# ltinphan/convex-mpc-unitree-go2

Measured on AMD Instinct MI355X. Metric: batched QP solves/sec (N=16, 4-leg friction cone) at 1/2/4/8 MI355X, higher is better.
Workload: dtype f32

## Files before the change

### convex-mpc-unitree-go2_amd/csrc/cmpc_condense.h

```cpp
#pragma once
#include "cmpc_instance.h"

namespace cmpc {

template <int NC>
__device__ __forceinline__ void condense_finish(Smem<NC>& s, f4 (&M)[Cfg<NC>::NTL], int n,
                                                float shift) {
  using C = Cfg<NC>;
  const int lane = opaque_lane();
  const int g = lane >> 4, c = lane & 15;
#pragma unroll
  for (int I = 0; I < C::TT; ++I) {
#pragma unroll
    for (int J = 0; J <= I; ++J) {
      if (J != I && 16 * I + 16 <= n) continue;
      f4 v = M[tile_index(I, J)];
      const int col = 16 * J + c;
#pragma unroll
      for (int q = 0; q < 4; ++q) {
        const int row = 16 * I + 4 * g + q;
        if (row >= n || col >= n) v[q] = (row == col) ? 1.f : 0.f;
        else if (row == col) v[q] += s.Rt[row] + shift;
      }
      M[tile_index(I, J)] = v;
    }
  }
  WSYNC();
}

__device__ __forceinline__ int lane_state(int c) {
  return ((c & 3) < 3) ? 3 * (c >> 2) + (c & 3) : -1;
}
template <class SM>
__device__ __forceinline__ void state_operands(SM& s, int g, int c, float (&aA)[3],
                                               float (&aT)[3], f4& q2) {
  const int sc = lane_state(c);
  q2 = f4{0.f, 0.f, 0.f, 0.f};
#pragma unroll
  for (int q = 0; q < 3; ++q) {
    const int r = 3 * g + q;
    aA[q] = (sc >= 0) ? s.A[sc * 12 + r] : 0.f;
    aT[q] = (sc >= 0) ? s.A[r * 12 + sc] : 0.f;
    q2[q] = (r == sc) ? s.Q2[r] : 0.f;
  }
}

template <class SM>
__device__ __forceinline__ void blockrow_C_chunk(SM& s, float* Cs, const f4& Pt, int J, int p0,
                                                 int p1, int n, int g, int c) {
  const int p = 16 * J + c;
  float bt[3];
#pragma unroll
  for (int q = 0; q < 3; ++q) bt[q] = s.Bt[p * kBS + 3 * g + q];
  f4 d = {0.f, 0.f, 0.f, 0.f};
#pragma unroll
  for (int q = 0; q < 3; ++q) d = mfma4(Pt[q], (p < n) ? bt[q] : 0.f, d);
  if (p >= p0 && p < p1) {
#pragma unroll
    for (int q = 0; q < 3; ++q) Cs[p * 12 + 3 * g + q] = d[q];
  }
}
__device__ __forceinline__ void blockrow_P_step(f4& Pt, const float (&aT)[3], const f4& q2) {
  f4 y = {0.f, 0.f, 0.f, 0.f}, z = {0.f, 0.f, 0.f, 0.f};
#pragma unroll
  for (int q = 0; q < 3; ++q) y = mfma4(Pt[q], aT[q], y);
#pragma unroll
  for (int q = 0; q < 3; ++q) z = mfma4(aT[q], y[q], z);
#pragma unroll
  for (int q = 0; q < 4; ++q) Pt[q] = z[q] + q2[q];
}

template <int NC>
__device__ __forceinline__ void condense_tiles_fwd(Smem<NC>& s, const KParams& P,
                                                   f4 (&M)[Cfg<NC>::NTL], int n, float shift) {
  using C = Cfg<NC>;
  const int lane = opaque_lane();
  const int g = lane >> 4, c = lane & 15;
  const int N = P.N;
  n = uniform(n);
#pragma unroll
  for (int t = 0; t < C::NTL; ++t) M[t] = f4{0.f, 0.f, 0.f, 0.f};
  float aA[3], q2[3];
  const int sc = lane_state(c);
#pragma unroll
  for (int q = 0; q < 3; ++q) {
    const int r = 3 * g + q;
    aA[q] = (sc >= 0) ? s.A[sc * 12 + r] : 0.f;
    q2[q] = s.Q2[r];
  }
  int kI[C::TT];
#pragma unroll
  for (int I = 0; I < C::TT; ++I) kI[I] = (16 * I < n) ? s.par[16 * I] : N;
  f4 Gd[C::TT];
#pragma unroll
  for (int J = 0; J < C::TT; ++J) Gd[J] = f4{0.f, 0.f, 0.f, 0.f};
  for (int t = 0; t < N; ++t) {
    if (t > 0) {
#pragma unroll
      for (int J = 0; J < C::TT; ++J) {
        if (kI[J] >= t) continue;
        f4 d = {0.f, 0.f, 0.f, 0.f};
#pragma unroll
        for (int q = 0; q < 3; ++q) d = mfma4(aA[q], Gd[J][q], d);
        Gd[J] = d;
      }
    }
    const int p0 = s.off[t], p1 = s.off[t + 1];
#pragma unroll
    for (int J = 0; J < C::TT; ++J) {
      if (16 * J + 15 < p0 || 16 * J >= p1) continue;
      const int p = 16 * J + c;
      if (p >= p0 && p < p1) {
        const float* bp = &s.Bt[p * kBS + 3 * g];
        Gd[J] = f4{bp[0], bp[1], bp[2], 0.f};
      }
    }
#pragma unroll
    for (int I = 0; I < C::TT; ++I) {
      if (kI[I] > t) continue;
      float a[3];
#pragma unroll
      for (int q = 0; q < 3; ++q) a[q] = q2[q] * Gd[I][q];
#pragma unroll
      for (int J = 0; J <= I; ++J) {
        f4 acc = M[tile_index(I, J)];
#pragma unroll
        for (int q = 0; q < 3; ++q) acc = mfma4(a[q], Gd[J][q], acc);
        M[tile_index(I, J)] = acc;
      }
    }
  }
  condense_finish<NC>(s, M, n, shift);
}

template <int NC>
__device__ __forceinline__ void mirror_diagonals(Smem<NC>& s, f4 (&M)[Cfg<NC>::NTL], int n, int N) {
  using C = Cfg<NC>;
  const int lane = opaque_lane();
  const int g = lane >> 4, c = lane & 15;
  WSYNC();
  float* T = s.G;
#pragma unroll
  for (int I = 0; I < C::TT; ++I) {
    if (16 * I >= n) continue;
    f4 v = M[tile_index(I, I)];
#pragma unroll
    for (int q = 0; q < 4; ++q) T[(4 * g + q) * 16 + c] = v[q];
    WSYNC();
    const int pc = 16 * I + c;
    const int kc = (pc < n) ? s.par[pc] : N;
#pragma unroll
    for (int q = 0; q < 4; ++q) {
      const int pr = 16 * I + 4 * g + q;
      const int kr = (pr < n) ? s.par[pr] : N;
      if (kc > kr) v[q] = T[c * 16 + 4 * g + q];
    }
    M[tile_index(I, I)] = v;
    WSYNC();
  }
}

template <int NC>
__device__ __forceinline__ void condense_tiles_bc(Smem<NC>& s, const KParams& P,
                                                  f4 (&M)[Cfg<NC>::NTL], int n, float shift) {
  using C = Cfg<NC>;
  const int lane = opaque_lane();
  const int g = lane >> 4, c = lane & 15;
  const int N = P.N;
  n = uniform(n);
#pragma unroll
  for (int t = 0; t < C::NTL; ++t) M[t] = f4{0.f, 0.f, 0.f, 0.f};
  float aA[3], aT[3];
  f4 q2;
  state_operands(s, g, c, aA, aT, q2);
  float* Cs = s.G;
  f4 Pt = q2;
  WSYNC();
  for (int i = N - 1; i >= 0; --i) {
    const int p0 = s.off[i], p1 = s.off[i + 1];
#pragma unroll
    for (int J = 0; J < C::TT; ++J) {
      if (16 * J + 15 < p0 || 16 * J >= p1) continue;
      blockrow_C_chunk(s, Cs, Pt, J, p0, p1, n, g, c);
    }
    if (i > 0) blockrow_P_step(Pt, aT, q2);
  }
  WSYNC();
  int kI[C::TT];
#pragma unroll
  for (int I = 0; I < C::TT; ++I) kI[I] = (16 * I < n) ? s.par[16 * I] : N;
  f4 Gd[C::TT];
#pragma unroll
  for (int J = 0; J < C::TT; ++J) Gd[J] = f4{0.f, 0.f, 0.f, 0.f};
  for (int t = 0; t < N; ++t) {
    if (t > 0) {
#pragma unroll
      for (int J = 0; J < C::TT; ++J) {
        if (kI[J] >= t) continue;
        f4 d = {0.f, 0.f, 0.f, 0.f};
#pragma unroll
        for (int q = 0; q < 3; ++q) d = mfma4(aA[q], Gd[J][q], d);
        Gd[J] = d;
      }
    }
    const int p0 = s.off[t], p1 = s.off[t + 1];
#pragma unroll
    for (int J = 0; J < C::TT; ++J) {
      if (16 * J + 15 < p0 || 16 * J >= p1) continue;
      const int p = 16 * J + c;
      if (p >= p0 && p < p1) {
        const float* bp = &s.Bt[p * kBS + 3 * g];
        Gd[J] = f4{bp[0], bp[1], bp[2], 0.f};
      }
    }
#pragma unroll
    for (int I = 0; I < C::TT; ++I) {
      if (16 * I + 15 < p0 || 16 * I >= p1) continue;
      const int p = 16 * I + c;
      float a[3] = {0.f, 0.f, 0.f};
      if (p >= p0 && p < p1) {
#pragma unroll
        for (int q = 0; q < 3; ++q) a[q] = Cs[p * 12 + 3 * g + q];
      }
#pragma unroll
      for (int J = 0; J <= I; ++J) {
        f4 acc = M[tile_index(I, J)];
#pragma unroll
        for (int q = 0; q < 3; ++q) acc = mfma4(a[q], Gd[J][q], acc);
        M[tile_index(I, J)] = acc;
      }
    }
  }
  mirror_diagonals<NC>(s, M, n, N);
  condense_finish<NC>(s, M, n, shift);
}

__device__ __forceinline__ void step_sums(int k, int N, float& S0, float& S1, float& S2) {
  S0 = (float)(N - k);
  S1 = (float)((N * (N - 1) - k * (k - 1)) >> 1);
  S2 = (float)(((N - 1) * N * (2 * N - 1) - (k - 1) * k * (2 * k - 1)) / 6);
}

template <int NC>
__device__ __forceinline__ void condense_tiles_nil(Smem<NC>& s, const KParams& P,
                                                   f4 (&M)[Cfg<NC>::NTL], int n, float shift) {
  using C = Cfg<NC>;
  const int lane = opaque_lane();
  const int g = lane >> 4, c = lane & 15;
  const int N = P.N;
  n = uniform(n);
  const int TA = (n + 15) >> 4;
#pragma unroll
  for (int t = 0; t < C::NTL; ++t) M[t] = f4{0.f, 0.f, 0.f, 0.f};
  float* Vs = s.G;
  {
    const int sc = lane_state(c);
    float aN[3];
#pragma unroll
    for (int q = 0; q < 3; ++q) {
      const int r = 3 * g + q;
      aN[q] = (sc >= 0) ? s.A[sc * 12 + r] - ((sc == r) ? 1.f : 0.f) : 0.f;
    }
    WSYNC();
#pragma unroll
    for (int J = 0; J < C::TT; ++J) {
      if (J >= TA) continue;
      const int p = 16 * J + c;
      float bt[3];
#pragma unroll
      for (int q = 0; q < 3; ++q) bt[q] = (p < n) ? s.Bt[p * kBS + 3 * g + q] : 0.f;
      f4 d = {0.f, 0.f, 0.f, 0.f};
#pragma unroll
      for (int q = 0; q < 3; ++q) d = mfma4(aN[q], bt[q], d);
#pragma unroll
      for (int q = 0; q < 3; ++q) Vs[p * 12 + 3 * g + q] = d[q];
    }
  }
  WSYNC();
  float q2[3];
#pragma unroll
  for (int q = 0; q < 3; ++q) q2[q] = s.Q2[3 * g + q];
  float uc[C::TT][3], vc[C::TT][3];
#pragma unroll
  for (int J = 0; J < C::TT; ++J) {
    const int p = 16 * J + c;
    const bool ok = J < TA && p < n;
    const float kf = ok ? (float)s.par[p] : 0.f;
#pragma unroll
    for (int q = 0; q < 3; ++q) {
      vc[J][q] = ok ? Vs[p * 12 + 3 * g + q] : 0.f;
      uc[J][q] = ok ? fmaf(-kf, vc[J][q], s.Bt[p * kBS + 3 * g + q]) : 0.f;
    }
  }
#pragma unroll
  for (int I = 0; I < C::TT; ++I) {
    if (I >= TA) continue;
    float x[3], y[3];
    {
      const int p = 16 * I + c;
      const bool ok = p < n;
      const int k = ok ? s.par[p] : 0;
      const float kf = (float)k;
      float S0, S1, S2;
      step_sums(k, N, S0, S1, S2);
#pragma unroll
      for (int q = 0; q < 3; ++q) {
        const float v = ok ? Vs[p * 12 + 3 * g + q] : 0.f;
        const float u = ok ? fmaf(-kf, v, s.Bt[p * kBS + 3 * g + q]) : 0.f;
        x[q] = q2[q] * fmaf(S0, u, S1 * v);
        y[q] = q2[q] * fmaf(S1, u, S2 * v);
      }
    }
#pragma unroll
    for (int J = 0; J <= I; ++J) {
      float u[3], v[3];
#pragma unroll
      for (int q = 0; q < 3; ++q) {
        u[q] = uc[J][q];
        v[q] = vc[J][q];
      }
      f4 acc = M[tile_index(I, J)];
#pragma unroll
      for (int q = 0; q < 3; ++q) acc = mfma4(x[q], u[q], acc);
#pragma unroll
      for (int q = 0; q < 3; ++q) acc = mfma4(y[q], v[q], acc);
      M[tile_index(I, J)] = acc;
    }
  }
  mirror_diagonals<NC>(s, M, n, N);
  condense_finish<NC>(s, M, n, shift);
}

template <class SM>
__device__ __forceinline__ bool nilpotent_step(SM& s) {
  const int lane = opaque_lane();
  WSYNC();
  bool nz = false;
#pragma unroll
  for (int e0 = 0; e0 < 144; e0 += 64) {
    const int e = e0 + lane;
    if (e < 144) {
      const int i = e / 12, j = e % 12;
      float acc = 0.f;
#pragma unroll
      for (int k = 0; k < 12; ++k) {
        const float nik = s.A[i * 12 + k] - ((i == k) ? 1.f : 0.f);
        const float nkj = s.A[k * 12 + j] - ((k == j) ? 1.f : 0.f);
        acc = fmaf(nik, nkj, acc);
      }
      nz |= acc != 0.f;
    }
  }
  return __any(nz) == 0;
}

template <int NC>
__device__ __forceinline__ void condense_tiles(Smem<NC>& s, const KParams& P,
                                               f4 (&M)[Cfg<NC>::NTL], int n, float shift,
                                               bool nil = false) {
  if (nil) {
    condense_tiles_nil<NC>(s, P, M, n, shift);
    return;
  }
  if constexpr (NC <= 128) {
    if (P.latency_mode) {
      condense_tiles_bc<NC>(s, P, M, n, shift);
      return;
    }
  }
  condense_tiles_fwd<NC>(s, P, M, n, shift);
}

}
```

### convex-mpc-unitree-go2_amd/csrc/cmpc_factor.h

```cpp
#pragma once
#include "cmpc_instance.h"

namespace cmpc {

constexpr int kSweepPipeMaxNC = 128;
template <int NC, int K, class SM>
__device__ __forceinline__ void sweep_publish(SM& s, const f4 (&M)[Cfg<NC>::NTL], int sub,
                                              int g, int c) {
  using C = Cfg<NC>;
  const int c0 = 4 * sub;
  const int pc = c - c0;
  const bool colw = pc >= 0 && pc < 4;
  if (colw) {
#pragma unroll
    for (int I = K; I < C::TT; ++I) {
      f4 m = M[tile_index(I, K)];
      if (I == K) {
#pragma unroll
        for (int q = 0; q < 4; ++q) m[q] -= (4 * g + q == c) ? 1.f : 0.f;
      }
#pragma unroll
      for (int q = 0; q < 4; ++q) s.pan[(16 * I + 4 * g + q) * 4 + pc] = m[q];
    }
  }
  WSYNC();
}

__device__ __forceinline__ void pivot_block(const float (&Dm)[16], int g, float& w0, float& w1,
                                            float& w2, float& w3, float& ig) {
  const bool g1 = g == 1, g2 = g == 2, g3 = g == 3;
  const float i0 = __builtin_amdgcn_rcpf(Dm[0]);
  const float l10 = Dm[4] * i0, l20 = Dm[8] * i0, l30 = Dm[12] * i0;
  const float i1 = __builtin_amdgcn_rcpf(Dm[5] - l10 * Dm[4]);
  const float u21 = Dm[9] - l20 * Dm[4], u31 = Dm[13] - l30 * Dm[4];
  const float l21 = u21 * i1, l31 = u31 * i1;
  const float i2 = __builtin_amdgcn_rcpf(Dm[10] - l20 * Dm[8] - l21 * u21);
  const float u32 = Dm[14] - l30 * Dm[8] - l31 * u21;
  const float l32 = u32 * i2;
  const float i3 = __builtin_amdgcn_rcpf(Dm[15] - l30 * Dm[12] - l31 * u31 - l32 * u32);
  const float n10 = -l10, n21 = -l21, n32 = -l32;
  const float n20 = l21 * l10 - l20, n31 = l32 * l21 - l31;
  const float n30 = -l30 - l31 * n10 - l32 * n20;
  w0 = g3 ? n30 : g2 ? n20 : g1 ? n10 : 1.f;
  w1 = g3 ? n31 : g2 ? n21 : g1 ? 1.f : 0.f;
  w2 = g3 ? n32 : g2 ? 1.f : 0.f;
  w3 = g3 ? 1.f : 0.f;
  ig = g3 ? i3 : g2 ? i2 : g1 ? i1 : i0;
}
__device__ __forceinline__ float panel_row(const f4& ph, float w0, float w1, float w2, float w3) {
  return fmaf(w3, ph[3], fmaf(w2, ph[2], fmaf(w1, ph[1], w0 * ph[0])));
}

template <int NC, int KMIN, class SM>
__device__ __forceinline__ void sweep_operands(SM& s, int k0, int g, int c,
                                               float (&a)[Cfg<NC>::TT], float (&b)[Cfg<NC>::TT]) {
  using C = Cfg<NC>;
  float Dm[16];
#pragma unroll
  for (int i = 0; i < 4; ++i) {
    const f4 rrow = *reinterpret_cast<const f4*>(&s.pan[(k0 + i) * 4]);
#pragma unroll
    for (int j = 0; j < 4; ++j) Dm[i * 4 + j] = (i == j) ? rrow[j] + 1.f : rrow[j];
  }
  f4 ph[C::TT];
#pragma unroll
  for (int I = KMIN; I < C::TT; ++I) ph[I] = *reinterpret_cast<const f4*>(&s.pan[(16 * I + c) * 4]);
  float w0, w1, w2, w3, ig;
  pivot_block(Dm, g, w0, w1, w2, w3, ig);
#pragma unroll
  for (int I = KMIN; I < C::TT; ++I) {
    const float yg = panel_row(ph[I], w0, w1, w2, w3);
    a[I] = -yg;
    b[I] = yg * ig;
  }
}

template <int NC, int Kc, bool CRIT, int KMIN>
__device__ __forceinline__ void sweep_mfma(f4 (&M)[Cfg<NC>::NTL], const float (&a)[Cfg<NC>::TT],
                                           const float (&b)[Cfg<NC>::TT], int TA) {
  using C = Cfg<NC>;
#pragma unroll
  for (int I = KMIN; I < C::TT; ++I) {
    if (I >= TA) continue;
#pragma unroll
    for (int J = KMIN; J <= I; ++J) {
      const bool crit = J == Kc && I >= Kc;
      if (crit != CRIT) continue;
      const int t = tile_index(I, J);
      M[t] = mfma4(a[I], b[J], M[t]);
    }
  }
}

template <int NC, int K>
__device__ __forceinline__ void sweep_diagfix(f4 (&M)[Cfg<NC>::NTL], int sub, int g, int c) {
  const int pc = c - 4 * sub;
  const bool roww = g == sub;
  f4& m = M[tile_index(K, K)];
#pragma unroll
  for (int q = 0; q < 4; ++q) m[q] -= (roww && pc == q) ? 2.f : 0.f;
}

template <int NC, int K, class SM>
__device__ __forceinline__ void sweep_block(SM& s, f4 (&M)[Cfg<NC>::NTL], int ng, int TA,
                                            int g, int c, float (&a)[Cfg<NC>::TT],
                                            float (&b)[Cfg<NC>::TT]) {
  using C = Cfg<NC>;
  constexpr int KM = K;
  if constexpr (K < C::TT) {
    if (4 * K < ng) {
      const int subs = (ng - 4 * K) < 4 ? (ng - 4 * K) : 4;
      for (int sub = 0; sub < subs - 1; ++sub) {
        sweep_mfma<NC, K, true, KM>(M, a, b, TA);
        sweep_diagfix<NC, K>(M, sub, g, c);
        sweep_publish<NC, K>(s, M, sub + 1, g, c);
        sweep_mfma<NC, K, false, KM>(M, a, b, TA);
        sweep_operands<NC, KM>(s, 16 * K + 4 * (sub + 1), g, c, a, b);
      }
      {
        const int sub = subs - 1;
        const bool has_next = 4 * (K + 1) < ng;
        sweep_mfma<NC, K + 1, true, KM>(M, a, b, TA);
        if constexpr (K + 1 < C::TT) {
          if (has_next) sweep_publish<NC, K + 1>(s, M, 0, g, c);
        }
        sweep_mfma<NC, K + 1, false, KM>(M, a, b, TA);
        sweep_diagfix<NC, K>(M, sub, g, c);
        if constexpr (K + 1 < C::TT) {
          if (has_next) sweep_operands<NC, K + 1>(s, 16 * (K + 1), g, c, a, b);
        }
      }
    }
    sweep_block<NC, K + 1>(s, M, ng, TA, g, c, a, b);
  }
}

template <int NC, int K, class SM>
__device__ __forceinline__ void sweep_block_plain(SM& s, f4 (&M)[Cfg<NC>::NTL], int ng, int TA,
                                                  int g, int c) {
  using C = Cfg<NC>;
  if constexpr (K < C::TT) {
    if (4 * K < ng) {
      const int subs = (ng - 4 * K) < 4 ? (ng - 4 * K) : 4;
      for (int sub = 0; sub < subs; ++sub) {
        float a[C::TT], b[C::TT];
        sweep_publish<NC, K>(s, M, sub, g, c);
        sweep_operands<NC, K>(s, 16 * K + 4 * sub, g, c, a, b);
        sweep_mfma<NC, -1, false, K>(M, a, b, TA);
        sweep_diagfix<NC, K>(M, sub, g, c);
      }
    }
    sweep_block_plain<NC, K + 1>(s, M, ng, TA, g, c);
  }
}

template <int NC, class SM>
__device__ __forceinline__ void ldl_tiles(SM& s, f4 (&M)[Cfg<NC>::NTL], int n) {
  using C = Cfg<NC>;
  const int lane = opaque_lane();
  const int g = lane >> 4, c = lane & 15;
  n = uniform(n);
  const int TA = (n + 15) >> 4;
#pragma unroll
  for (int I = 0; I < C::TT; ++I) {
    const f4 d = M[tile_index(I, I)];
#pragma unroll
    for (int q = 0; q < 4; ++q) {
      const int p = 16 * I + c;
      if (4 * g + q == c) s.ds[p] = (p < n && d[q] > 0.f) ? rsqrtf(d[q]) : 1.f;
    }
  }
  WSYNC();
#pragma unroll
  for (int I = 0; I < C::TT; ++I) {
    const f4 ri = *reinterpret_cast<const f4*>(&s.ds[16 * I + 4 * g]);
#pragma unroll
    for (int J = 0; J <= I; ++J) {
      const float cj = s.ds[16 * J + c];
      f4& m = M[tile_index(I, J)];
#pragma unroll
      for (int q = 0; q < 4; ++q) m[q] *= ri[q] * cj;
    }
  }
  const int ng = (n + 3) >> 2;
  if constexpr (NC <= kSweepPipeMaxNC) {
    if (ng > 0) {
      float a[C::TT], b[C::TT];
      sweep_publish<NC, 0>(s, M, 0, g, c);
      sweep_operands<NC, 0>(s, 0, g, c, a, b);
      sweep_block<NC, 0>(s, M, ng, TA, g, c, a, b);
    }
  } else {
    sweep_block_plain<NC, 0>(s, M, ng, TA, g, c);
  }
#pragma unroll
  for (int I = 0; I < C::TT; ++I) {
    const f4 ri = *reinterpret_cast<const f4*>(&s.ds[16 * I + 4 * g]);
    f4 rinv;
#pragma unroll
    for (int q = 0; q < 4; ++q) rinv[q] = 1.f / ri[q];
#pragma unroll
    for (int J = 0; J <= I; ++J) {
      const float cj = s.ds[16 * J + c];
      f4& m = M[tile_index(I, J)];
#pragma unroll
      for (int q = 0; q < 4; ++q) m[q] *= (J < I) ? rinv[q] * cj : -(ri[q] * cj);
    }
  }
}

template <int NC, class SM>
__device__ __forceinline__ void ldl_apply(SM& s, const f4 (&M)[Cfg<NC>::NTL], int n,
                                          const float* in, float* out) {
  using C = Cfg<NC>;
  CMPC_T0(t_sv);
  const int lane = opaque_lane();
  const int g = lane >> 4, c = lane & 15;
  n = uniform(n);
  const int TA = (n + 15) >> 4;
  WSYNC();
  float zc[C::TT];
  float bc[C::TT];
#pragma unroll
  for (int I = 0; I < C::TT; ++I) bc[I] = 0.f;
#pragma unroll
  for (int I = 0; I < C::TT; ++I) {
    if (I >= TA) {
      if (c == 0) *reinterpret_cast<f4*>(&out[16 * I + 4 * g]) = f4{0.f, 0.f, 0.f, 0.f};
      continue;
    }
    f4 zr = *reinterpret_cast<const f4*>(&in[16 * I + 4 * g]);
    if (I > 0) {
      f2 r01 = {0.f, 0.f}, r23 = {0.f, 0.f};
#pragma unroll
      for (int J = 0; J < I; ++J) {
        const f4 m = M[tile_index(I, J)];
        const f2 zj = {zc[J], zc[J]};
        r01 = __builtin_elementwise_fma(f2{m[0], m[1]}, zj, r01);
        r23 = __builtin_elementwise_fma(f2{m[2], m[3]}, zj, r23);
      }
      zr[0] -= row16_sum(r01[0]);
      zr[1] -= row16_sum(r01[1]);
      zr[2] -= row16_sum(r23[0]);
      zr[3] -= row16_sum(r23[1]);
    }
#pragma unroll
    for (int q = 0; q < 4; ++q) zr[q] = (16 * I + 4 * g + q < n) ? zr[q] : 0.f;
    if (c == 0) *reinterpret_cast<f4*>(&out[16 * I + 4 * g]) = zr;
    WSYNC();
    zc[I] = out[16 * I + c];
  }
#pragma unroll
  for (int I = C::TT - 1; I >= 0; --I) {
    if (I >= TA) continue;
    const f4 zr = *reinterpret_cast<const f4*>(&out[16 * I + 4 * g]);
    const f4 d = M[tile_index(I, I)];
    const float t =
        fmaf(d[3], zr[3], fmaf(d[2], zr[2], fmaf(d[1], zr[1], fmaf(d[0], zr[0], -bc[I]))));
    float xc = col4_sum(t);
    xc = (16 * I + c < n) ? xc : 0.f;
    WSYNC();
    if (g == 0) out[16 * I + c] = xc;
    if (I == 0) break;
    WSYNC();
    const f4 xr = *reinterpret_cast<const f4*>(&out[16 * I + 4 * g]);
#pragma unroll
    for (int J = 0; J < I; ++J) {
      const f4 m = M[tile_index(I, J)];
      bc[J] = fmaf(m[3], xr[3], fmaf(m[2], xr[2], fmaf(m[1], xr[1], fmaf(m[0], xr[0], bc[J]))));
    }
  }
  WSYNC();
  CMPC_ACC(3, t_sv);
  CMPC_CNT(13, 1);
}

template <int NC>
__device__ __forceinline__ void park_store(float* __restrict__ park, const f4 (&M)[Cfg<NC>::NTL]) {
  const int lane = opaque_lane();
#pragma unroll
  for (int t = 0; t < Cfg<NC>::NTL; ++t)
    *reinterpret_cast<f4*>(&park[t * 256 + lane * 4]) = M[t];
}

template <int NC>
__device__ __forceinline__ void park_load(const float* __restrict__ park, f4 (&M)[Cfg<NC>::NTL]) {
  const int lane = opaque_lane();
  asm volatile("s_waitcnt vmcnt(0)\n\tbuffer_inv sc1" ::: "memory");
#pragma unroll
  for (int t = 0; t < Cfg<NC>::NTL; ++t)
    M[t] = *reinterpret_cast<const f4*>(&park[t * 256 + lane * 4]);
}

}
```

### convex-mpc-unitree-go2_amd/csrc/cmpc_instance.h

```cpp
#pragma once
#include "cmpc_device.h"
#include "cmpc_wave_prims.h"

namespace cmpc {

constexpr int kMaxN = 16;
constexpr int kMaxP = 12 * kMaxN;
constexpr int kMaxTri = 4 * kMaxN;

template <int NC>
struct Cfg {
  static_assert(NC % 16 == 0, "bin capacity must be a multiple of 16");
  static constexpr int TT = NC / 16;
  static constexpr int NTL = TT * (TT + 1) / 2;
  static constexpr int THREADS = 64;
  static constexpr int SLAB = NTL * 256;
  static constexpr int WPE = (4 * NTL <= 150) ? 2 : 1;
};

constexpr int kRefineExtra = 4;
constexpr float kRefineRate = 0.5f;
constexpr int kBackoffCap = 3;
constexpr int kLateRepairs = 3;
constexpr int kRepairTop = 2;
constexpr int kStableGrow = 3;
constexpr bool kRhoLowHeavy = true;
constexpr int kFailMem = 4;
constexpr int kTryMem = 8;
constexpr float kLooseTol = 5.f;
constexpr float kFaceErr = 2.f;
constexpr float kLooseFace = 2.5f;
constexpr float kCertFace = 5e-5f;
constexpr int kAmbRefine = 2;
constexpr float kAmbBand = 5.f;
constexpr float kAmbConverged = 1e-2f;
constexpr float kFailRho = 4.f;

constexpr int kBS = 12;

template <int NC>
struct Smem {
#ifdef CMPC_STAMPS
  unsigned long long st[32];
#endif
  alignas(16) float Bt[NC * kBS];
  alignas(16) float Rt[NC];
  alignas(16) float x[NC];
  alignas(16) float z[NC];
  alignas(16) float y[NC];
  alignas(16) float v[NC];
  union {
    struct {
      alignas(16) float g[NC];
      alignas(16) float r[NC];
      alignas(16) float dl[NC];
      alignas(16) float ds[NC];
      alignas(16) float pan[NC * 4];
      float H[kMaxP];
      float E[kMaxP];
      float L[kMaxP];
    };
    alignas(16) float G[NC * 12];
  };
  float D[kMaxP];
  float Dt[kMaxP];
  float A[144];
  float Q2[12];
  float R2[12];
  int par[NC];
  int off[kMaxN + 1];
  int nil;
  int tri[kMaxTri];
  int tri_of[kMaxTri];
  int8_t tcnt[kMaxTri];
  int8_t code[kMaxTri];
  int8_t pcode[kMaxTri];
  int fpk[kMaxTri];
  uint8_t fpat[kFailMem][kMaxTri];
  uint8_t tpat[kTryMem][kMaxTri];
};

__device__ __forceinline__ constexpr int tile_index(int I, int J) { return (I * (I + 1)) / 2 + J; }

struct Terrain {
  float mu, fz_min;
};
__device__ __forceinline__ Terrain instance_terrain(const KParams& P, const Inputs& in, int64_t b) {
  Terrain T{P.mu, P.fz_min};
  if (in.mu) T.mu = uniformf(in.mu[b]);
  if (in.fz_min) T.fz_min = uniformf(in.fz_min[b]);
  return T;
}
__device__ __forceinline__ bool terrain_valid(const Terrain& T) {
  return T.mu > 0.f && isfinite(T.mu) && isfinite(T.fz_min);
}

template <int NC, int W>
struct TeamCfg {
  static constexpr int TT = NC / 16;
  static constexpr int NPAIR = TT / 2;
  static constexpr int PPW = (NPAIR + W - 1) / W;
  static constexpr int SLOTS = W == 1 ? TT * (TT + 1) / 2 : PPW * (TT + 1);
  static constexpr int SLAB = W * SLOTS * 256;
  static_assert(W == 1 || TT % 2 == 0, "team mode pairs tile columns");
};

}
```

### convex-mpc-unitree-go2_amd/csrc/cmpc_polish.h

```cpp
#pragma once
#include "cmpc_factor.h"

namespace cmpc {

__device__ __forceinline__ int project(float a, float b, float c, float mu, float fzmin,
                                       float& px, float& py, float& pz) {
  const float Aa = fabsf(a), Bb = fabsf(b);
  const float lo = fminf(Aa, Bb), hi = fmaxf(Aa, Bb);
  const float z1 = (c + mu * (Aa + Bb)) / (1.f + 2.f * mu * mu);
  const float z2 = (c + mu * hi) / (1.f + mu * mu);
  float zz = (mu * z1 < lo) ? z1 : ((mu * z2 < hi) ? z2 : c);
  int code = 0;
  if (zz < fzmin) { zz = fzmin; code |= 1; }
  const float lim = mu * zz;
  if (a > lim) { px = lim; code |= 2; } else if (a < -lim) { px = -lim; code |= 4; } else px = a;
  if (b > lim) { py = lim; code |= 8; } else if (b < -lim) { py = -lim; code |= 16; } else py = b;
  pz = zz;
  return code;
}

__device__ __forceinline__ int faces_at(float fx, float fy, float fz, float mu, float fz_min,
                                        float slack) {
  const float tz = 1e-5f * fmaxf(fz, 1.f), lim = mu * fz - slack;
  int code = (fz <= fz_min + tz) ? 1 : 0;
// ... 186 lines not shown
  const int code = owns ? s.code[lane] : 0;
  const int kl = owns ? s.tri[lane] : 0;
  const int k = kl >> 2, leg = kl & 3;
  const int sx = (code & 2) ? 1 : ((code & 4) ? -1 : 0);
  const int sy = (code & 8) ? 1 : ((code & 16) ? -1 : 0);
  const bool zl = (code & 1) != 0;
  if (owns) {
    const int pk = s.fpk[lane];
    const int px = pk & 255, py = (pk >> 8) & 255, pz = (pk >> 16) & 255;
    fz = zl ? fzmin : s.v[pz];
    fx = (sx == 0) ? s.v[px] : sx * mu * fz;
    fy = (sy == 0) ? s.v[py] : sy * mu * fz;
    const float* Bk = Bg + k * 144 + 3 * leg;
    float ax = 0.f, ay = 0.f, az = 0.f;
#pragma unroll
    for (int r = 0; r < 12; ++r) {
      const float lr = s.L[12 * k + r];
      ax = fmaf(Bk[r * 12], lr, ax);
      ay = fmaf(Bk[r * 12 + 1], lr, ay);
      az = fmaf(Bk[r * 12 + 2], lr, az);
    }
    gx = ax + s.R2[3 * leg] * fx;
    gy = ay + s.R2[3 * leg + 1] * fy;
    gz = az + s.R2[3 * leg + 2] * fz;
  }
  const float gs = wave_max(fmaxf(fabsf(gx), fmaxf(fabsf(gy), fabsf(gz))));
  const float us = wave_max(fmaxf(1.f, fmaxf(fabsf(fx), fmaxf(fabsf(fy), fabsf(fz)))));
  const float tol_d = P.polish_tol * gs, tol_p = P.polish_tol * us;
  const bool prec = uniform(s.nil) != 0;
  float tfx = tol_d, tfy = tol_d, tfz = tol_d;
  if (prec && owns) {
    const float fe = kFaceErr * P.polish_tol * us;
    tfx = fminf(tol_d, fe * s.R2[3 * leg]);
    tfy = fminf(tol_d, fe * s.R2[3 * leg + 1]);
    tfz = fminf(tol_d, fe * s.R2[3 * leg + 2]);
  }
  bool ok = true, am = false, dec = false;
  int nc = 0;
  float v = 0.f, csq = 0.f;
  if (owns) {
    const float lx = sx ? -sx * gx : 0.f;
    const float ly = sy ? -sy * gy : 0.f;
    const float l0 = gz - mu * (lx + ly);
    const float ta = kAmbBand * tol_d;
    am = prec && ((sx && lx < ta) || (sy && ly < ta) || (zl && l0 < ta));
    nc = code;
    if (sx && lx < -tfx) { ok = false; nc &= ~6; dec = dec || lx < -ta; }
    if (sy && ly < -tfy) { ok = false; nc &= ~24; dec = dec || ly < -ta; }
    if (zl && l0 < -tfz) { ok = false; nc &= ~1; dec = dec || l0 < -ta; }
    if (!sx && fabsf(fx) > mu * fz + tol_p) { ok = false; nc |= (fx > 0.f) ? 2 : 4; dec = true; }
    if (!sy && fabsf(fy) > mu * fz + tol_p) { ok = false; nc |= (fy > 0.f) ? 8 : 16; dec = true; }
    if (!zl && fz < fzmin - tol_p) { ok = false; nc |= 1; dec = true; }
    if (!(isfinite(fx) && isfinite(fy) && isfinite(fz))) { ok = false; dec = true; }
    const float ig = 1.f / fmaxf(gs, 1e-30f), iu = 1.f / us;
    v = fmaxf(fmaxf(sx ? -lx * ig : 0.f, sy ? -ly * ig : 0.f), zl ? -l0 * ig : 0.f);
    v = fmaxf(v, fmaxf(sx ? 0.f : (fabsf(fx) - mu * fz) * iu, sy ? 0.f : (fabsf(fy) - mu * fz) * iu));
    v = fmaxf(v, zl ? 0.f : (fzmin - fz) * iu);
    const bool fin = isfinite(fx) && isfinite(fy) && isfinite(fz);
    TRACE_IF(tr >= 0 && (v > 0.f || (sx && lx < tfx) || (sy && ly < tfy) || (zl && l0 < tfz)),
             "[%d]       tri %d k %d leg %d code %d f %g %g %g  l %g %g %g  tol %g %g %g  v %g\n",
             tr, lane, k, leg, code, fx, fy, fz, lx, ly, l0, tfx, tfy, tfz, v);
    lok = fin && v <= kLooseTol * P.polish_tol;
    if (prec)
      lok = lok && !(sx && lx < -kLooseFace * tfx) && !(sy && ly < -kLooseFace * tfy) &&
            !(zl && l0 < -kLooseFace * tfz);
    s.dl[3 * lane] = fx;
    s.dl[3 * lane + 1] = fy;
    s.dl[3 * lane + 2] = fz;
    const float nx = sx ? fminf(lx, 0.f) : 0.f, ny = sy ? fminf(ly, 0.f) : 0.f;
    const float nz = zl ? fminf(l0, 0.f) : 0.f;
    const float cx = nx * sx, cy = ny * sy, cz = -mu * (nx + ny) - nz;
    csq = fmaf(cx, cx, fmaf(cy, cy, cz * cz));
    if (!isfinite(csq)) csq = INFINITY;
  }
  s.r[lane] = owns ? csq : 0.f;
  if (lane == 0) s.r[64] = us;
  if (top > 0) {
    const bool cand = owns && nc != code;
    float key = cand ? (isfinite(v) ? v : INFINITY) : -1.f;
    bool sel = false;
    const int ncand = __popcll(__ballot(cand));
    const int kk = max(top, (ncand + 1) >> 1);
    for (int r = 0; r < kk; ++r) {
      const float m = wave_max(key);
      if (!(m > 0.f)) break;
      const unsigned long long bal = __ballot(key == m);
      if (lane == __builtin_ctzll(bal)) {
        sel = true;
        key = -1.f;
      }
    }
    if (cand && !sel) nc = code;
  }
  if (owns) s.tcnt[lane] = nc;
  PolishCheck res;
  res.changed = __any(owns && nc != code) != 0;
  res.amb = __any(am) != 0;
  res.decisive = __any(dec) != 0;
  res.vworst = wave_max((owns && isfinite(v)) ? v : (owns ? 1e30f : 0.f));
  const bool step_ok = step <= P.polish_tol * us;
  res.converged = step_ok;
  res.loose = (__all(lok) != 0) && step_ok;
  const bool all_ok = (__all(ok) != 0) && step_ok;
  res.ok = all_ok;
  if (all_ok && owns) {
    float px, py, pz;
    project(fx, fy, fz, mu, fzmin, px, py, pz);
    s.x[3 * lane] = px;
    s.x[3 * lane + 1] = py;
    s.x[3 * lane + 2] = pz;
  }
  return res;
}

template <int NC>
__device__ __forceinline__ bool certified_faces(Smem<NC>& s, float r2_min) {
  const int lane = opaque_lane();
  WSYNC();
  const float c2 = wave_sum(s.r[lane]);
  return uniformf(sqrtf(c2)) <= kCertFace * r2_min * uniformf(s.r[64]);
}

#ifndef CMPC_DD_CAP
#define CMPC_DD_CAP 6
#endif
__host__ __device__ constexpr int dd_max(int NC) {
  return (5 * NC + kMaxP - 32) / NC < CMPC_DD_CAP ? (5 * NC + kMaxP - 32) / NC : CMPC_DD_CAP;
}
template <int NC>
__device__ __forceinline__ float* dd_w(Smem<NC>& s, int j) { return s.ds + j * NC; }
template <int NC>
__device__ __forceinline__ float* dd_meta(Smem<NC>& s) { return s.H + kMaxP - 32; }

template <int NC, class MT>
__device__ __forceinline__ bool face_downdate(Smem<NC>& s, const Terrain& T, const MT& M, int n,
                                              int ntri, int& nadd) {
  static_assert(dd_max(NC) >= 1 && dd_max(NC) <= 8, "the meta block holds 8 faces");
  static_assert(offsetof(Smem<NC>, H) == offsetof(Smem<NC>, ds) + 5 * NC * sizeof(float),
                "ds, pan and H are one slab");
  const int lane = opaque_lane();
  n = uniform(n);
  float* meta = dd_meta(s);
  WSYNC();
  int F;
  {
    const bool owns = lane < ntri;
    const int oc = owns ? s.code[lane] : 0, nc = owns ? s.tcnt[lane] : 0;
    const int add = nc & ~oc;
    const int cnt = face_count(add);
    int j = nadd + wave_excl_scan4(cnt);
    F = uniform(wave_total4(cnt));
    if (nadd + F > dd_max(NC)) return false;
    if (owns && add) {
      const float mu = T.mu, fzmin = T.fz_min;
      const int pk = s.fpk[lane];
      const int px = pk & 255, py = (pk >> 8) & 255, pz = (pk >> 16) & 255;
      if (add & 1) {
        meta[8 + j] = __int_as_float(pz | (pz << 8)); meta[16 + j] = 0.f; meta[24 + j] = fzmin; ++j;
      }
#pragma unroll
      for (int ax = 0; ax < 2; ++ax) {
        const int bits = ax ? (add & 24) : (add & 6);
        if (!bits) continue;
        const int pa = ax ? py : px;
        const float sg = (bits & (ax ? 8 : 2)) ? 1.f : -1.f;
        if (pz != 255) {
          meta[8 + j] = __int_as_float(pa | (pz << 8)); meta[16 + j] = -sg * mu; meta[24 + j] = 0.f;
        } else {
          meta[8 + j] = __int_as_float(pa | (pa << 8)); meta[16 + j] = 0.f; meta[24 + j] = sg * mu * fzmin;
        }
        ++j;
      }
    }
  }
  WSYNC();
  const int j1 = nadd + F;
  for (int j = nadd; j < j1; ++j) {
    const int q = __float_as_int(meta[8 + j]);
    const int p1 = q & 255, p2 = (q >> 8) & 255;
    const float cf = meta[16 + j], cv = meta[24 + j];
    for (int p = lane; p < NC; p += 64) s.r[p] = (p == p1) ? 1.f : (p == p2) ? cf : 0.f;
    float* w = dd_w(s, j);
    ldl_apply<NC>(s, M, n, s.r, w);
    for (int i = 0; i < j; ++i) {
      const float* wi = dd_w(s, i);
      const float t = fmaf(cf, wi[p2], wi[p1]) * meta[i];
      for (int p = lane; p < n; p += 64) w[p] = fmaf(-t, wi[p], w[p]);
      WSYNC();
    }
    const float d = fmaf(cf, w[p2], w[p1]);
    if (!(d > 0.f) || !isfinite(d)) return false;
    const float id = 1.f / d;
    const float res = (fmaf(cf, s.v[p2], s.v[p1]) - cv) * id;
    WSYNC();
    for (int p = lane; p < n; p += 64) s.v[p] = fmaf(-res, w[p], s.v[p]);
    if (lane == 0) meta[j] = id;
    WSYNC();
  }
  nadd = j1;
  return true;
}

template <int NC>
__device__ __forceinline__ void dd_apply(Smem<NC>& s, int n, int nadd, const float* gin,
                                         float* dl) {
  const int lane = opaque_lane();
  const float* meta = dd_meta(s);
  n = uniform(n);
  WSYNC();
  float sj[dd_max(NC)];
#pragma unroll
  for (int j = 0; j < dd_max(NC); ++j) {
    if (j >= nadd) break;
    const float* w = dd_w(s, j);
    float part = 0.f;
    for (int p = lane; p < n; p += 64) part = fmaf(w[p], gin[p], part);
    sj[j] = wave_sum(part) * meta[j];
  }
  for (int p = lane; p < n; p += 64) {
    float acc = dl[p];
#pragma unroll
    for (int j = 0; j < dd_max(NC); ++j) {
      if (j >= nadd) break;
      acc = fmaf(-sj[j], dd_w(s, j)[p], acc);
    }
    dl[p] = acc;
  }
  WSYNC();
}

}
```

### convex-mpc-unitree-go2_amd/csrc/cmpc_team.hip

```cpp
#pragma once
#include "cmpc_condense.h"
#include "cmpc_factor.h"

namespace cmpc {

enum : int { kOpExit = 0, kOpFactor = 1, kOpSymv = 2, kOpParkStore = 3, kOpParkLoad = 4 };

template <int NC, int W>
struct TeamSmem {
  int cmd[2][4];
  alignas(16) float ds[NC];
  union {
    alignas(16) float pan[2][NC * 4];
    struct {
      alignas(16) float partR[NC / 32][NC];
      alignas(16) float partC[NC];
    };
    alignas(16) float scr[W][512];
  };
};

template <int NC, int W>
__device__ __forceinline__ bool team_slot(int w, int j, int l, int& I, int& J) {
  using T = TeamCfg<NC, W>;
// ... 241 lines not shown
        for (int q = 0; q < 3; ++q) acc = mfma4(x[q], u[q], acc);
#pragma unroll
        for (int q = 0; q < 3; ++q) acc = mfma4(y[q], v[q], acc);
        M[j * (TT + 1) + l] = acc;
      }
    }
    CMPC_ACC(17, t_f1);
  } else {
  {
    f4 Pt = q2;
    for (int i = N - 1; i >= 0; --i) {
      const int p0 = s.off[i], p1 = s.off[i + 1];
#pragma unroll
      for (int J = 0; J < TT; ++J) {
        if (J % W != w) continue;
        if (16 * J + 15 < p0 || 16 * J >= p1) continue;
        blockrow_C_chunk(s, Cs, Pt, J, p0, p1, n, g, c);
      }
      if (i > 0) blockrow_P_step(Pt, aT, q2);
    }
  }
  team_barrier();
  CMPC_ACC(16, t_f0);
  CMPC_T0(t_f1);
  {
    f4 Gd[T::PPW][2];
    int kJ[T::PPW][2];
#pragma unroll
    for (int j = 0; j < T::PPW; ++j) {
#pragma unroll
      for (int h = 0; h < 2; ++h) {
        const int pr = w + j * W;
        const int J = h ? TT - 1 - pr : pr;
        Gd[j][h] = f4{0.f, 0.f, 0.f, 0.f};
        kJ[j][h] = (pr < T::NPAIR && 16 * J < n) ? uniform(s.par[16 * J]) : N;
      }
    }
    for (int t = 0; t < N; ++t) {
      const int p0 = uniform(s.off[t]), p1 = uniform(s.off[t + 1]);
      const int Ia = min(p0 >> 4, TT - 1), Ib = (p1 > p0) ? (p1 - 1) >> 4 : Ia;
      f4 alo = {0.f, 0.f, 0.f, 0.f}, ahi = {0.f, 0.f, 0.f, 0.f};
#pragma unroll
      for (int q = 0; q < 3; ++q) {
        alo[q] = Cs[(16 * Ia + c) * 12 + 3 * g + q];
        ahi[q] = Cs[(16 * Ib + c) * 12 + 3 * g + q];
      }
      f4 bn[T::PPW][2];
#pragma unroll
      for (int j = 0; j < T::PPW; ++j) {
#pragma unroll
        for (int h = 0; h < 2; ++h) {
          const int pr = w + j * W;
          const int J = (pr < T::NPAIR) ? (h ? TT - 1 - pr : pr) : 0;
          bn[j][h] = f4{0.f, 0.f, 0.f, 0.f};
#pragma unroll
          for (int q = 0; q < 3; ++q) bn[j][h][q] = s.Bt[(16 * J + c) * kBS + 3 * g + q];
        }
      }
      pin(alo);
      pin(ahi);
#pragma unroll
      for (int j = 0; j < T::PPW; ++j) {
        pin(bn[j][0]);
        pin(bn[j][1]);
      }
      {
        const int pa = 16 * Ia + c, pb_ = 16 * Ib + c;
        const bool ma = pa >= p0 && pa < p1, mb = pb_ >= p0 && pb_ < p1;
#pragma unroll
        for (int q = 0; q < 3; ++q) {
          alo[q] = ma ? alo[q] : 0.f;
          ahi[q] = mb ? ahi[q] : 0.f;
        }
      }
#pragma unroll
      for (int j = 0; j < T::PPW; ++j) {
        const int pr = w + j * W;
        if (pr >= T::NPAIR) continue;
#pragma unroll
        for (int h = 0; h < 2; ++h) {
          const int J = h ? TT - 1 - pr : pr;
          if (t > 0 && kJ[j][h] < t) {
            f4 d = {0.f, 0.f, 0.f, 0.f};
#pragma unroll
            for (int q = 0; q < 3; ++q) d = mfma4(aA[q], Gd[j][h][q], d);
            Gd[j][h] = d;
          }
          const int p = 16 * J + c;
          if (p >= p0 && p < p1) Gd[j][h] = bn[j][h];
        }
#pragma unroll
        for (int l = 0; l <= TT; ++l) {
          int I, J;
          team_slot<NC, W>(w, j, l, I, J);
          if (I != Ia && I != Ib) continue;
          if (p1 == p0) continue;
          const f4 a = (I == Ia) ? alo : ahi;
          const f4 gj = (l < TT - pr) ? Gd[j][0] : Gd[j][1];
          f4 acc = M[j * (TT + 1) + l];
#pragma unroll
          for (int q = 0; q < 3; ++q) acc = mfma4(a[q], gj[q], acc);
          M[j * (TT + 1) + l] = acc;
        }
      }
    }
  }
  CMPC_ACC(17, t_f1);
  }
  CMPC_T0(t_f2);
  float* scr = ts.scr[w];
#pragma unroll
  for (int j = 0; j < T::PPW; ++j) {
    const int pr = w + j * W;
    if (pr >= T::NPAIR) continue;
    const int base = j * (TT + 1);
    const int Jd[2] = {pr, TT - 1 - pr};
    const int ld[2] = {0, TT - pr};
    f4 v[2], tr[2];
    int kc[2], kr[2][4];
    float rt[2];
#pragma unroll
    for (int h = 0; h < 2; ++h) v[h] = M[base + ld[h]];
    WSYNC();
#pragma unroll
    for (int h = 0; h < 2; ++h) {
#pragma unroll
      for (int q = 0; q < 4; ++q) scr[256 * h + (4 * g + q) * 16 + c] = v[h][q];
    }
    WSYNC();
#pragma unroll
    for (int h = 0; h < 2; ++h) {
      const int I = Jd[h];
#pragma unroll
      for (int q = 0; q < 4; ++q) tr[h][q] = scr[256 * h + c * 16 + 4 * g + q];
      kc[h] = s.par[16 * I + c];
#pragma unroll
      for (int q = 0; q < 4; ++q) kr[h][q] = s.par[16 * I + 4 * g + q];
      rt[h] = s.Rt[16 * I + c];
    }
    WSYNC();
#pragma unroll
    for (int h = 0; h < 2; ++h) {
      const int I = Jd[h];
      const int pc = 16 * I + c;
      const int kcv = (pc < n) ? kc[h] : N;
      f4 m = v[h];
#pragma unroll
      for (int q = 0; q < 4; ++q) {
        const int row = 16 * I + 4 * g + q;
        const int krv = (row < n) ? kr[h][q] : N;
        if (16 * I < n && kcv > krv) m[q] = tr[h][q];
        if (row >= n || pc >= n) m[q] = (row == pc) ? 1.f : 0.f;
        else if (row == pc) m[q] += rt[h] + shift;
        if (4 * g + q == c) ts.ds[pc] = (pc < n && m[q] > 0.f) ? rsqrtf(m[q]) : 1.f;
      }
      M[base + ld[h]] = m;
    }
#pragma unroll
    for (int l = 0; l <= TT; ++l) {
      int I, J;
      team_slot<NC, W>(w, j, l, I, J);
      if (I == J) continue;
      f4& m = M[base + l];
      const int col = 16 * J + c;
#pragma unroll
      for (int q = 0; q < 4; ++q) {
        const int row = 16 * I + 4 * g + q;
        if (row >= n || col >= n) m[q] = 0.f;
      }
    }
  }
  team_barrier();
  CMPC_ACC(18, t_f2);
  CMPC_T0(t_f3);
  team_scale<NC, W>(ts, M, w, g, c, 1.f);
  const int ng = (n + 3) >> 2;
  if constexpr (WV >= 0) {
#pragma unroll
    for (int K = 0; K < TT; ++K) {
      if (4 * K >= ng) continue;
      const int subs = (ng - 4 * K) < 4 ? (ng - 4 * K) : 4;
      for (int sub = 0; sub < subs; ++sub) team_sweep_step<NC, W, WV>(s, ts, M, w, K, sub, g, c);
    }
  } else {
    for (int kk = 0; kk < ng; ++kk) team_sweep_step<NC, W, WV>(s, ts, M, w, kk >> 2, kk & 3, g, c);
  }
  CMPC_ACC(19, t_f3);
  team_scale<NC, W>(ts, M, w, g, c, -1.f);
}

template <int NC, int W, int WV>
__device__ __forceinline__ void team_symv_part(TeamSmem<NC, W>& ts,
                                               const f4 (&M)[TeamCfg<NC, W>::SLOTS], int n,
                                               const float* in, int w_rt) {
  using T = TeamCfg<NC, W>;
  const int w = (WV >= 0) ? WV : uniform(w_rt);
  constexpr int TT = T::TT;
  const int lane = opaque_lane();
  const int g = lane >> 4, c = lane & 15;
  n = uniform(n);
#pragma unroll
  for (int j = 0; j < T::PPW; ++j) {
    const int pr = w + j * W;
    if (pr >= T::NPAIR) continue;
    const int J0 = pr, J1 = TT - 1 - pr;
    float xc0, xc1;
    f4 xr[TT];
    {
      const float v0 = in[16 * J0 + c], v1 = in[16 * J1 + c];
      xc0 = (16 * J0 + c < n) ? v0 : 0.f;
      xc1 = (16 * J1 + c < n) ? v1 : 0.f;
    }
#pragma unroll
    for (int r = 0; r < TT; ++r) {
      const int I = min(pr + r, TT - 1);
      xr[r] = *reinterpret_cast<const f4*>(&in[16 * I + 4 * g]);
#pragma unroll
      for (int q = 0; q < 4; ++q) xr[r][q] = (16 * I + 4 * g + q < n) ? xr[r][q] : 0.f;
    }
    pin(xc0);
    pin(xc1);
#pragma unroll
    for (int r = 0; r < TT; ++r) pin(xr[r]);
    float cacc0 = 0.f, cacc1 = 0.f;
#pragma unroll
    for (int r = 0; r < TT; ++r) {
      const int I = pr + r;
      if (I >= TT) break;
      const f4 m0 = M[j * (TT + 1) + r];
      f4 racc;
#pragma unroll
      for (int q = 0; q < 4; ++q) racc[q] = m0[q] * xc0;
      if (I > J0) {
        float cp = 0.f;
#pragma unroll
        for (int q = 0; q < 4; ++q) cp = fmaf(m0[q], xr[r][q], cp);
        cacc0 += cp;
      }
      if (I >= J1) {
        const f4 m1 = M[j * (TT + 1) + I + 1];
#pragma unroll
        for (int q = 0; q < 4; ++q) racc[q] = fmaf(m1[q], xc1, racc[q]);
        if (I > J1) {
          float cp = 0.f;
#pragma unroll
          for (int q = 0; q < 4; ++q) cp = fmaf(m1[q], xr[r][q], cp);
          cacc1 += cp;
        }
      }
      f4 rs;
#pragma unroll
      for (int q = 0; q < 4; ++q) rs[q] = row16_sum(racc[q]);
      if (c == 0) *reinterpret_cast<f4*>(&ts.partR[pr][16 * I + 4 * g]) = rs;
    }
    const float cs0 = col4_sum(cacc0), cs1 = col4_sum(cacc1);
    if (g == 0) {
      ts.partC[16 * J0 + c] = cs0;
      ts.partC[16 * J1 + c] = cs1;
    }
  }
}

template <int NC, int W>
__device__ __forceinline__ void team_symv_reduce(TeamSmem<NC, W>& ts, int n, float* out) {
  constexpr int NPAIR = NC / 32;
  const int lane = opaque_lane();
  n = uniform(n);
  const int TA = (n + 15) >> 4;
  for (int p = lane; p < NC; p += 64) {
    const int I = p >> 4;
    float acc = ts.partC[p];
#pragma unroll
    for (int pr = 0; pr < NPAIR; ++pr) {
      const float v = ts.partR[pr][p];
      acc += (pr <= I) ? v : 0.f;
    }
    out[p] = (I < TA) ? acc : 0.f;
  }
  WSYNC();
}

template <int NC, int W, int WV>
__device__ __forceinline__ void team_park_store(float* __restrict__ park,
                                                const f4 (&M)[TeamCfg<NC, W>::SLOTS], int w_rt) {
  const int w = (WV >= 0) ? WV : uniform(w_rt);
  const int lane = opaque_lane();
  float* base = park + (size_t)w * TeamCfg<NC, W>::SLOTS * 256;
#pragma unroll
  for (int t = 0; t < TeamCfg<NC, W>::SLOTS; ++t)
    *reinterpret_cast<f4*>(&base[t * 256 + lane * 4]) = M[t];
}

template <int NC, int W, int WV>
__device__ __forceinline__ void team_park_load(const float* __restrict__ park,
                                               f4 (&M)[TeamCfg<NC, W>::SLOTS], int w_rt) {
  const int w = (WV >= 0) ? WV : uniform(w_rt);
  const int lane = opaque_lane();
  const float* base = park + (size_t)w * TeamCfg<NC, W>::SLOTS * 256;
  asm volatile("s_waitcnt vmcnt(0)\n\tbuffer_inv sc1" ::: "memory");
#pragma unroll
  for (int t = 0; t < TeamCfg<NC, W>::SLOTS; ++t)
    M[t] = *reinterpret_cast<const f4*>(&base[t * 256 + lane * 4]);
}

template <int NC, int W>
__device__ __forceinline__ void team_issue(TeamSmem<NC, W>& ts, int& seq, int op, int a0, int a1,
                                           int a2) {
// ... 92 lines not shown
```

Baseline: 8.703 million.

## Streamline condense finish, batch diagonal mirroring, and precompute reciprocal scales

Several micro-optimizations across the condense and LDL factor paths. Diagonal padding and shift become branch-free selects, and the shift term is hoisted per tile row. Diagonal tiles are mirrored in batches through the G slab so fewer wave syncs are needed, with vectorized par/transpose loads made possible by aligning par. The nilpotent condense no longer zeroes all tiles up front and reuses cached operands. Reciprocals of the ds scales are computed once into pan instead of per tile, and diagonal rsqrt stores use a single selected element. The changes add shared-memory traffic and syncs in the factor path, and an empty asm barrier is placed on fzmin to steer codegen.

```diff
diff --git a/convex-mpc-unitree-go2_amd/csrc/cmpc_condense.h b/convex-mpc-unitree-go2_amd/csrc/cmpc_condense.h
--- a/convex-mpc-unitree-go2_amd/csrc/cmpc_condense.h
+++ b/convex-mpc-unitree-go2_amd/csrc/cmpc_condense.h
@@ -11,6 +11,7 @@
   const int g = lane >> 4, c = lane & 15;
 #pragma unroll
   for (int I = 0; I < C::TT; ++I) {
+    const float rs = s.Rt[16 * I + c] + shift;
 #pragma unroll
     for (int J = 0; J <= I; ++J) {
       if (J != I && 16 * I + 16 <= n) continue;
@@ -19,8 +20,14 @@
 #pragma unroll
       for (int q = 0; q < 4; ++q) {
         const int row = 16 * I + 4 * g + q;
-        if (row >= n || col >= n) v[q] = (row == col) ? 1.f : 0.f;
-        else if (row == col) v[q] += s.Rt[row] + shift;
+        const bool pad = row >= n || col >= n;
+        if (J == I) {
+          const bool dg = 4 * g + q == c;
+          const float dv = v[q] + rs;
+          v[q] = pad ? (dg ? 1.f : 0.f) : (dg ? dv : v[q]);
+        } else {
+          v[q] = pad ? 0.f : v[q];
+        }
       }
       M[tile_index(I, J)] = v;
     }
@@ -136,26 +143,41 @@
 template <int NC>
 __device__ __forceinline__ void mirror_diagonals(Smem<NC>& s, f4 (&M)[Cfg<NC>::NTL], int n, int N) {
   using C = Cfg<NC>;
+  constexpr int kFit = 12 * NC / 256, kBatches = (C::TT + kFit - 1) / kFit;
+  constexpr int BT = (C::TT + kBatches - 1) / kBatches;
+  static_assert(BT >= 1 && BT * 256 <= 12 * NC, "the batch fits the G slab");
+  typedef int i4 __attribute__((ext_vector_type(4)));
   const int lane = opaque_lane();
   const int g = lane >> 4, c = lane & 15;
   WSYNC();
   float* T = s.G;
 #pragma unroll
-  for (int I = 0; I < C::TT; ++I) {
-    if (16 * I >= n) continue;
-    f4 v = M[tile_index(I, I)];
-#pragma unroll
-    for (int q = 0; q < 4; ++q) T[(4 * g + q) * 16 + c] = v[q];
+  for (int I0 = 0; I0 < C::TT; I0 += BT) {
+    if (16 * I0 >= n) continue;
+#pragma unroll
+    for (int I = I0; I < I0 + BT && I < C::TT; ++I) {
+      if (16 * I >= n) continue;
+      const f4 v = M[tile_index(I, I)];
+#pragma unroll
+      for (int q = 0; q < 4; ++q) T[256 * (I - I0) + (4 * g + q) * 16 + c] = v[q];
+    }
     WSYNC();
-    const int pc = 16 * I + c;
-    const int kc = (pc < n) ? s.par[pc] : N;
-#pragma unroll
-    for (int q = 0; q < 4; ++q) {
-      const int pr = 16 * I + 4 * g + q;
-      const int kr = (pr < n) ? s.par[pr] : N;
-      if (kc > kr) v[q] = T[c * 16 + 4 * g + q];
-    }
-    M[tile_index(I, I)] = v;
+#pragma unroll
+    for (int I = I0; I < I0 + BT && I < C::TT; ++I) {
+      if (16 * I >= n) continue;
+      f4 v = M[tile_index(I, I)];
+      const int pc = 16 * I + c;
+      const int kc = (pc < n) ? s.par[pc] : N;
+      const i4 kr4 = *reinterpret_cast<const i4*>(&s.par[16 * I + 4 * g]);
+      const f4 tr = *reinterpret_cast<const f4*>(&T[256 * (I - I0) + c * 16 + 4 * g]);
+#pragma unroll
+      for (int q = 0; q < 4; ++q) {
+        const int pr = 16 * I + 4 * g + q;
+        const int kr = (pr < n) ? kr4[q] : N;
+        v[q] = (kc > kr) ? tr[q] : v[q];
+      }
+      M[tile_index(I, I)] = v;
+    }
     WSYNC();
   }
 }
@@ -250,8 +272,6 @@
   const int N = P.N;
   n = uniform(n);
   const int TA = (n + 15) >> 4;
-#pragma unroll
-  for (int t = 0; t < C::NTL; ++t) M[t] = f4{0.f, 0.f, 0.f, 0.f};
   float* Vs = s.G;
   {
     const int sc = lane_state(c);
@@ -294,19 +314,22 @@
   }
 #pragma unroll
   for (int I = 0; I < C::TT; ++I) {
-    if (I >= TA) continue;
+    if (I >= TA) {
+#pragma unroll
+      for (int J = 0; J <= I; ++J) M[tile_index(I, J)] = f4{0.f, 0.f, 0.f, 0.f};
+      continue;
+    }
     float x[3], y[3];
     {
       const int p = 16 * I + c;
       const bool ok = p < n;
       const int k = ok ? s.par[p] : 0;
-      const float kf = (float)k;
       float S0, S1, S2;
       step_sums(k, N, S0, S1, S2);
 #pragma unroll
       for (int q = 0; q < 3; ++q) {
-        const float v = ok ? Vs[p * 12 + 3 * g + q] : 0.f;
-        const float u = ok ? fmaf(-kf, v, s.Bt[p * kBS + 3 * g + q]) : 0.f;
+        const float v = vc[I][q];
+        const float u = uc[I][q];
         x[q] = q2[q] * fmaf(S0, u, S1 * v);
         y[q] = q2[q] * fmaf(S1, u, S2 * v);
       }
@@ -319,7 +342,7 @@
         u[q] = uc[J][q];
         v[q] = vc[J][q];
       }
-      f4 acc = M[tile_index(I, J)];
+      f4 acc = {0.f, 0.f, 0.f, 0.f};
 #pragma unroll
       for (int q = 0; q < 3; ++q) acc = mfma4(x[q], u[q], acc);
 #pragma unroll
diff --git a/convex-mpc-unitree-go2_amd/csrc/cmpc_factor.h b/convex-mpc-unitree-go2_amd/csrc/cmpc_factor.h
--- a/convex-mpc-unitree-go2_amd/csrc/cmpc_factor.h
+++ b/convex-mpc-unitree-go2_amd/csrc/cmpc_factor.h
@@ -2,6 +2,11 @@
 #include "cmpc_instance.h"
 
 namespace cmpc {
+
+__device__ __forceinline__ float diag_element(const f4& d, int c) {
+  const int qs = c & 3;
+  return qs == 0 ? d[0] : qs == 1 ? d[1] : qs == 2 ? d[2] : d[3];
+}
 
 constexpr int kSweepPipeMaxNC = 128;
 template <int NC, int K, class SM>
@@ -163,12 +168,10 @@
   const int TA = (n + 15) >> 4;
 #pragma unroll
   for (int I = 0; I < C::TT; ++I) {
-    const f4 d = M[tile_index(I, I)];
-#pragma unroll
-    for (int q = 0; q < 4; ++q) {
-      const int p = 16 * I + c;
-      if (4 * g + q == c) s.ds[p] = (p < n && d[q] > 0.f) ? rsqrtf(d[q]) : 1.f;
-    }
+    const float dg = diag_element(M[tile_index(I, I)], c);
+    const int p = 16 * I + c;
+    const float r = (p < n && dg > 0.f) ? rsqrtf(dg) : 1.f;
+    if ((c >> 2) == g) s.ds[p] = r;
   }
   WSYNC();
 #pragma unroll
@@ -193,15 +196,23 @@
   } else {
     sweep_block_plain<NC, 0>(s, M, ng, TA, g, c);
   }
+  float* rinvs = s.pan;
+  WSYNC();
+  const int lane_r = opaque_lane();
+  const int g_r = lane_r >> 4, c_r = lane_r & 15;
+#pragma unroll
+  for (int p0 = 0; p0 < NC; p0 += 64) {
+    const int p = p0 + lane_r;
+    if (p < NC) rinvs[p] = 1.f / s.ds[p];
+  }
+  WSYNC();
 #pragma unroll
   for (int I = 0; I < C::TT; ++I) {
-    const f4 ri = *reinterpret_cast<const f4*>(&s.ds[16 * I + 4 * g]);
-    f4 rinv;
-#pragma unroll
-    for (int q = 0; q < 4; ++q) rinv[q] = 1.f / ri[q];
+    const f4 ri = *reinterpret_cast<const f4*>(&s.ds[16 * I + 4 * g_r]);
+    const f4 rinv = *reinterpret_cast<const f4*>(&rinvs[16 * I + 4 * g_r]);
 #pragma unroll
     for (int J = 0; J <= I; ++J) {
-      const float cj = s.ds[16 * J + c];
+      const float cj = s.ds[16 * J + c_r];
       f4& m = M[tile_index(I, J)];
 #pragma unroll
       for (int q = 0; q < 4; ++q) m[q] *= (J < I) ? rinv[q] * cj : -(ri[q] * cj);
diff --git a/convex-mpc-unitree-go2_amd/csrc/cmpc_instance.h b/convex-mpc-unitree-go2_amd/csrc/cmpc_instance.h
--- a/convex-mpc-unitree-go2_amd/csrc/cmpc_instance.h
+++ b/convex-mpc-unitree-go2_amd/csrc/cmpc_instance.h
@@ -67,7 +67,7 @@
   float A[144];
   float Q2[12];
   float R2[12];
-  int par[NC];
+  alignas(16) int par[NC];
   int off[kMaxN + 1];
   int nil;
   int tri[kMaxTri];
diff --git a/convex-mpc-unitree-go2_amd/csrc/cmpc_polish.h b/convex-mpc-unitree-go2_amd/csrc/cmpc_polish.h
--- a/convex-mpc-unitree-go2_amd/csrc/cmpc_polish.h
+++ b/convex-mpc-unitree-go2_amd/csrc/cmpc_polish.h
@@ -362,7 +362,9 @@
     F = uniform(wave_total4(cnt));
     if (nadd + F > dd_max(NC)) return false;
     if (owns && add) {
-      const float mu = T.mu, fzmin = T.fz_min;
+      const float mu = T.mu;
+      float fzmin = T.fz_min;
+      asm volatile("" : "+v"(fzmin));
       const int pk = s.fpk[lane];
       const int px = pk & 255, py = (pk >> 8) & 255, pz = (pk >> 16) & 255;
       if (add & 1) {
diff --git a/convex-mpc-unitree-go2_amd/csrc/cmpc_team.hip b/convex-mpc-unitree-go2_amd/csrc/cmpc_team.hip
--- a/convex-mpc-unitree-go2_amd/csrc/cmpc_team.hip
+++ b/convex-mpc-unitree-go2_amd/csrc/cmpc_team.hip
@@ -417,7 +417,11 @@
         if (16 * I < n && kcv > krv) m[q] = tr[h][q];
         if (row >= n || pc >= n) m[q] = (row == pc) ? 1.f : 0.f;
         else if (row == pc) m[q] += rt[h] + shift;
-        if (4 * g + q == c) ts.ds[pc] = (pc < n && m[q] > 0.f) ? rsqrtf(m[q]) : 1.f;
+      }
+      {
+        const float dg = diag_element(m, c);
+        const float r = (pc < n && dg > 0.f) ? rsqrtf(dg) : 1.f;
+        if ((c >> 2) == g) ts.ds[pc] = r;
       }
       M[base + ld[h]] = m;
     }
```

Result: faster. 9.491 million, median of 6 (+9.1%).
